# wuji3/visiondk

Hardware: AMD Instinct MI355X
Metric: images/sec fwd+bwd+optimizer step (ViT-B/16, bs=256 per GPU) (higher is better)
Workload: dtype fp16; 1 GPU; ViT-B/16 ICT, synthetic ImageNet-1k 224x224, random-init weights (reference re-init), per-GPU batch 256, CE label_smoothing 0.05, SGD 0.006/0.937/5e-4, clip 10, EMA on rank 0; global_batch=256, parallelism=dp1

## Files before the change

visiondk_amd/csrc/vit_engine.hip:

```cpp
#include <hip/hip_runtime.h>
#include <stdlib.h>
#include <stdio.h>
#include <string.h>
#include "vdk_device.h"
#include "vdk_host.h"
#include "vdk_gemm.h"

extern "C" {
int vdk_layernorm_fwd(const float*, int64_t, int32_t, int32_t, const float*, const float*, float, void*, int64_t, int32_t, float*, float*, void*);
int vdk_layernorm_bwd_workspace_bytes(int32_t, int32_t, size_t*);
int vdk_layernorm_bwd(const void*, int64_t, int32_t, const float*, int64_t, const float*, const float*, const float*, const float*, int64_t,
                      int32_t, int32_t, float*, int64_t, void*, int64_t, float*, float*, void*, size_t, void*);
int vdk_reduce_rows_f32(const float*, int64_t, int32_t, int64_t, float*, float, void*);
int vdk_colsum_bf16_workspace_bytes(int32_t, int32_t, size_t*);
int vdk_colsum_bf16(const void*, int64_t, int32_t, int32_t, float*, void*, size_t, void*);
int vdk_attention_fwd(const void*, int64_t, void*, int64_t, float*, int32_t, int32_t, int32_t, int32_t, float, void*);
int vdk_attention_bwd(const void*, int64_t, const void*, const void*, int64_t, const float*, void*, int64_t, float*, int32_t, int32_t, int32_t,
                      int32_t, float, void*);
int vdk_attention_fwd_dt(const void*, int64_t, void*, int64_t, float*, int32_t, int32_t, int32_t, int32_t, float, int32_t, void*);
int vdk_attention_bwd_dt(const void*, int64_t, const void*, const void*, int64_t, const float*, void*, int64_t, float*, int32_t, int32_t, int32_t, int32_t, float, int32_t, void*);
int vdk_attention_bwd_cs(const void*, int64_t, const void*, const void*, int64_t, const float*, void*, int64_t, float*, int32_t, int32_t, int32_t, int32_t, float, int32_t, float*, int32_t*,
                         void*);
int vdk_patchify_bf16(const float*, int32_t, int32_t, int32_t, int32_t, int32_t, void*, int32_t, void*);
int vdk_cls_rows(float*, int64_t, int32_t, int32_t, const float*, const float*, void*);
int vdk_cast_f32_bf16(const float*, void*, int64_t, void*);
int vdk_transpose_cast_f32_bf16(const float*, int64_t, int32_t, int32_t, void*, int64_t, int32_t, void*);
int vdk_gemm_f32_nt(const VdkGemmF32Desc*, void*);
int vdk_gemm_a_colsum_rows(int32_t, int32_t, int32_t);
int vdk_softmax_rows_f32(float*, int64_t, int64_t, int32_t, float, void*);
int vdk_patchify_f32(const float*, int32_t, int32_t, int32_t, int32_t, int32_t, float*, void*);
int vdk_quant_fp8(const void*, int32_t, int64_t, const float*, void*, int32_t, float*, void*);
int vdk_fp8_scale_update(float*, float*, float*, int32_t, int32_t, float, void*);
int vdk_gemm_fp8_nt(const VdkGemmDesc*, int32_t, int32_t, const float*, const float*, void*);
int vdk_gemm_fp8_nt_q8(const VdkGemmDesc*, int32_t, int32_t, const float*, const float*, void*, int64_t, int32_t, const float*, float*, void*);
int vdk_layernorm_fwd_q8(const float*, int64_t, int32_t, int32_t, const float*, const float*, float, void*, int64_t, float*, float*, void*, int64_t, int32_t, const float*, float*, void*);
}


static thread_local int t_opf = VDK_OPF_BF16;
#define DT16 (t_opf ? VDK_F16 : VDK_BF16)
static bool gelu_saved_grad() {
  static const int v = [] { const char* e = getenv("VDK_VIT_GELU_SAVED_GRAD"); return e ? atoi(e) : -1; }();
  return v < 0 ? t_opf != 0 : v != 0;
}
#define ACT_FC1 (gelu_saved_grad() ? VDK_ACT_GELU_SAVE_GRAD : VDK_ACT_GELU)
#define ACT_DFC2 (gelu_saved_grad() ? VDK_ACT_MUL_AUX : VDK_ACT_DGELU)

static inline int64_t up(int64_t x, int64_t a) { return (x + a - 1) / a * a; }

struct VitDims {
  int B, img, ps, Cin, D, L, H, M, C, Cp, np, N, T, Kraw, Kpe, Tp, Bp, cls, pre , fp8, opf ;
  float eps;
};
static int vit_dims(const VdkVitConfig* c, VitDims* d) {
  if (!c) return vdk_fail(VDK_EINVAL, "vit: null config");
  d->B = c->batch; d->img = c->img_size; d->ps = c->patch_size; d->Cin = c->in_chans; d->D = c->dim; d->L = c->depth;
  d->H = c->heads; d->M = c->mlp_dim; d->C = c->num_classes; d->eps = c->ln_eps;
  if (d->B <= 0 || d->img <= 0 || d->ps <= 0 || d->img % d->ps || d->Cin <= 0 || d->D <= 0 || d->L <= 0 || d->H <= 0 || d->M <= 0 || d->C < 0)
    return vdk_fail(VDK_EINVAL, "vit: bad config value");
  if (d->D != d->H * 64) return vdk_fail(VDK_EUNSUPPORTED, "vit: head_dim must be 64 (dim == 64 * heads)");
  if ((d->D & 7) || (d->M & 7)) return vdk_fail(VDK_EUNSUPPORTED, "vit: dim and mlp_dim must be multiples of 8");
  d->Kraw = d->Cin * d->ps * d->ps;
  d->Kpe = (int)up(d->Kraw, 8);
  d->np = (d->img / d->ps) * (d->img / d->ps);
  d->cls = c->no_class_token ? 0 : 1;
  d->pre = c->pre_norm ? 1 : 0;
  if (d->pre && c->fp8) return vdk_fail(VDK_EUNSUPPORTED, "vit: pre_norm and the fp8 mode are not combined");
  if (!d->cls && d->C > 0) return vdk_fail(VDK_EUNSUPPORTED, "vit: no_class_token is feature mode only (num_classes == 0)");
  d->N = d->np + d->cls;
// ... 144 lines not shown
  if (s > 64) s = 64;
  if (s < 1) s = 1;
  return s;
}
static int vit_plan(const VitDims& d, WsPlan* w) {
  size_t cur = 0;
  const size_t T = d.T, D = d.D, M = d.M, L = d.L;
  w->patches = w_take(cur, (size_t)d.B * d.np * d.Kpe * 2);
  w->pepad = w->dwpe = 0;
  if (d.Kraw != d.Kpe) { w->pepad = w_take(cur, D * d.Kpe * 2); w->dwpe = w_take(cur, D * d.Kpe * 4); }
  w->X = w_take(cur, (2 * L + 1) * T * D * 4);
  w->xe = w->pstats = 0;
  if (d.pre) { w->xe = w_take(cur, T * D * 4); w->pstats = w_take(cur, 2 * T * 4); }
  w->stats = w_take(cur, (L * 4 * T + 2 * T) * 4);
  w->s_h = T * D * 2; w->s_qkv = T * 3 * D * 2; w->s_lse = (size_t)d.B * d.H * d.N * 4; w->s_u = T * M * 2;
  w->h1 = w_take(cur, L * w->s_h); w->qkv = w_take(cur, L * w->s_qkv); w->lse = w_take(cur, L * w->s_lse);
  w->o = w_take(cur, L * w->s_h); w->h2 = w_take(cur, L * w->s_h); w->u = w_take(cur, L * w->s_u); w->g = w_take(cur, L * w->s_u);
  w->hf = w_take(cur, (size_t)d.Bp * D * 2);
  w->dxa = w_take(cur, T * D * 4); w->dxm = w_take(cur, T * D * 4);
  size_t big = M > 3 * D ? M : 3 * D;
  for (int i = 0; i < 3; ++i) w->dxab[i] = w_take(cur, T * D * 2);
  for (int i = 0; i < 2; ++i) {
    w->dxmb[i] = w_take(cur, T * D * 2);
    w->du[i] = w_take(cur, T * M * 2); w->dqkv[i] = w_take(cur, T * 3 * D * 2);
  }
  w->dsm = w_take(cur, T * D * 2);
  w->dvec = w_take(cur, w->s_lse);
  size_t trows = big > (size_t)d.Cp ? big : (size_t)d.Cp;
  if (trows < (size_t)d.Kpe) trows = d.Kpe;
  size_t tcols = d.Tp > d.Bp ? d.Tp : d.Bp;
  w->tA = w_take(cur, trows * tcols * 2); w->tB = w_take(cur, trows * tcols * 2);
  size_t sl = 0;
  {
    int sh[5][3] = {{(int)M, (int)D, d.T}, {(int)D, (int)M, d.T}, {3 * (int)D, (int)D, d.T}, {(int)D, (int)D, d.T}, {(int)D, d.Kpe, d.B * d.np}};
    for (auto& s : sh) {
      int k1 = wgrad_splitk(s[0], s[1], s[2]), k2 = wgrad_splitk_tn(s[0], s[1], s[2]);
      size_t b = (size_t)(k1 > k2 ? k1 : k2) * s[0] * s[1] * 4; if (b > sl) sl = b;
    }
  }
  w->slabs_bytes = sl; w->slabs = w_take(cur, sl);
  vdk_layernorm_bwd_workspace_bytes(d.T, d.D, &w->lnws_bytes); w->lnws_bytes = (w->lnws_bytes + 255) & ~(size_t)255; w->lnws = w_take(cur, 2 * w->lnws_bytes);
  size_t cs = (size_t)((tcols + 63) / 64) * trows * 4;
  { size_t cs2 = 0; vdk_colsum_bf16_workspace_bytes(d.T, (int)trows, &cs2); if (cs2 > cs) cs = cs2; }
  { size_t cs3 = (size_t)2 * ((d.T + 255) / 256) * trows * 4; if (cs3 > cs) cs = cs3; }
  w->csws_bytes = (cs + 255) & ~(size_t)255; w->csws = w_take(cur, 5 * w->csws_bytes);
  w->dhf = w_take(cur, (size_t)d.B * D * 2);
  w->dposall = w_take(cur, (size_t)d.N * D * 4);
  w->a8 = d.fp8 ? w_take(cur, T * (M > 3 * D ? M : 3 * D)) : 0;
  w->a8b = d.fp8 ? w_take(cur, T * M) : 0;
  w->total = cur;
  return VDK_OK;
}

#define RC(x) do { int rc_ = (x); if (rc_) return rc_; } while (0)

static bool cls_tail_on(const VitDims& d) {
  const char* e = getenv("VDK_VIT_CLS_TAIL");
  return d.C > 0 && d.cls && !d.fp8 && !(e && e[0] == '0');
}

struct F8 {
  int mode; unsigned char* w8; unsigned char* wt8; float* amax; float* sc; float* si; unsigned char* a8; unsigned char* a8b;
};
static int f8_init(const VdkVitConfig* cfg, const VitDims& d, const PLayout& p, F8* f, unsigned char* a8, unsigned char* a8b) {
  f->mode = d.fp8; f->a8 = a8; f->a8b = a8b;
  if (!d.fp8) return VDK_OK;
  if (!cfg->fp8_w || !cfg->fp8_state) return vdk_fail(VDK_EINVAL, "vit: fp8 mode without fp8_w / fp8_state");
  if (a8 && d.T < 256) return vdk_fail(VDK_EUNSUPPORTED, "vit: the fp8 mode needs batch * tokens >= 256");
  f->w8 = (unsigned char*)cfg->fp8_w; f->wt8 = f->w8 + p.total;
  const int S = 12 * d.L;
  f->amax = cfg->fp8_state; f->sc = f->amax + S; f->si = f->sc + S;
  return VDK_OK;
}
static int f8_quant(hipStream_t s, const F8& f, const void* x, int xdt, long n, int slot, int fmt, unsigned char* out, int force_current = 0) {
  if (f.mode == 2 || force_current) {
    RC(vdk_quant_fp8(x, xdt, n, nullptr, nullptr, fmt, f.amax + slot, s));
    RC(vdk_fp8_scale_update(f.amax + slot, f.sc + slot, f.si + slot, 1, fmt, 1.0f, s));
  }
  return vdk_quant_fp8(x, xdt, n, f.sc + slot, out, fmt, f.amax + slot, s);
}
static bool f8_fused(const F8& f) {
  const char* e = getenv("VDK_FP8_FUSED_QUANT");
  return f.mode == 1 && !(e && e[0] == '0');
}
static int gemm8(hipStream_t s, const F8& f, const void* a, int slot_a, int a_fmt, const unsigned char* w8, int slot_w, int64_t ldb, void* Cc, int64_t ldc, int M, int N,
                 int K, int cdt, const float* bias, const float* res, int64_t ldr, int act, void* aux, int64_t ldaux, const unsigned char* a_pre = nullptr, int q8_slot = -1,
                 int q8_fmt = 0, float* c_colsum = nullptr) {
  if (!a_pre) RC(f8_quant(s, f, a, VDK_BF16, (long)M * K, slot_a, a_fmt, f.a8));
  VdkGemmDesc g = {};
  g.A = a_pre ? a_pre : f.a8; g.lda = K; g.B = w8; g.ldb = ldb; g.C = Cc; g.ldc = ldc; g.M = M; g.N = N; g.K = K; g.c_dtype = cdt; g.bias = bias; g.residual = res; g.ldr = ldr;
  g.act = act; g.aux = aux; g.ldaux = ldaux; g.alpha = 1.0f; g.splitk = 1; g.c_colsum = c_colsum;
// ... 117 lines not shown
                    float* logits, void* stream_) {
  hipStream_t s = (hipStream_t)stream_;
  VitDims d; RC(vit_dims(cfg, &d));
  PLayout p; RC(vit_layout(d, &p));
  WsPlan w; RC(vit_plan(d, &w));
  if (!x || !params || !wb16 || !ws || !logits) return vdk_fail(VDK_EINVAL, "vdk_vit_forward: null pointer");
  if (ws_bytes < w.total) return vdk_fail(VDK_EWORKSPACE, "vdk_vit_forward: workspace too small");
  t_opf = d.opf;
  char* base = (char*)ws;
  const bf16_t* wb = (const bf16_t*)wb16;
  const int T = d.T, D = d.D, M = d.M;
  float* X = (float*)(base + w.X);
  float* stats = (float*)(base + w.stats);
  const size_t XS = (size_t)T * D;

  bf16_t* patches = (bf16_t*)(base + w.patches);
  RC(vdk_patchify_16(x, d.B, d.Cin, d.img, d.img, d.ps, patches, d.Kpe, t_opf, s));
  const bf16_t* pew = wb + p.pe_w;
  if (d.Kraw != d.Kpe) {
    RC(vdk_cast_pad_rows(params + p.pe_w, d.Kraw, D, d.Kraw, base + w.pepad, d.Kpe, s, t_opf));
    pew = (const bf16_t*)(base + w.pepad);
  }
  float* const X0 = d.pre ? (float*)(base + w.xe) : X;
  RC(gemm(s, patches, d.Kpe, pew, d.Kpe, X0, D, d.B * d.np, D, d.Kpe, VDK_F32, params + p.pe_b, params + p.pos, D, VDK_ACT_NONE,
          nullptr, 0, 1, d.cls ? d.np : -d.np, nullptr, 0));
  if (d.cls) RC(vdk_cls_rows(X0, (int64_t)d.N * D, d.B, D, params + p.cls, params + p.pos, s));
  if (d.pre) {
    float* ps = (float*)(base + w.pstats);
    RC(vdk_layernorm_fwd(X0, D, T, D, params + p.npre_w, params + p.npre_b, d.eps, X, D, VDK_F32, ps, ps + T, s));
  }

  const float scale = 0.125f;
  F8 f8; RC(f8_init(cfg, d, p, &f8, (unsigned char*)(base + w.a8), (unsigned char*)(base + w.a8b)));
  const bool cls_tail = cls_tail_on(d);
  for (int l = 0; l < d.L; ++l) {
    const PLayout::Blk& b = p.blk[l];
    float* xin = X + (size_t)(2 * l) * XS; float* xmid = xin + XS; float* xout = xmid + XS;
    float* mean1 = stats + (size_t)l * 4 * T; float* rstd1 = mean1 + T; float* mean2 = rstd1 + T; float* rstd2 = mean2 + T;
    bf16_t* h1 = (bf16_t*)(base + w.h1 + l * w.s_h); bf16_t* qkv = (bf16_t*)(base + w.qkv + l * w.s_qkv);
    float* lse = (float*)(base + w.lse + l * w.s_lse); bf16_t* o = (bf16_t*)(base + w.o + l * w.s_h);
    bf16_t* h2 = (bf16_t*)(base + w.h2 + l * w.s_h); bf16_t* u = (bf16_t*)(base + w.u + l * w.s_u); bf16_t* g = (bf16_t*)(base + w.g + l * w.s_u);
    if (f8.mode) {
      const int sl = 12 * l;
      const bool fl = f8_fused(f8) && D > 128 && D <= 1024, fq = f8_fused(f8) && (M % 64) == 0;
      if (fl) RC(vdk_layernorm_fwd_q8(xin, D, T, D, params + b.n1w, params + b.n1b, d.eps, h1, D, mean1, rstd1, f8.a8, D, 0, f8.sc + sl + 0, f8.amax + sl + 0, s));
      else RC(vdk_layernorm_fwd(xin, D, T, D, params + b.n1w, params + b.n1b, d.eps, h1, D, VDK_BF16, mean1, rstd1, s));
      RC(gemm8(s, f8, h1, sl + 0, 0, f8.w8 + b.qkv_w, sl + 4, D, qkv, 3 * D, T, 3 * D, D, VDK_BF16, params + b.qkv_b, nullptr, 0, VDK_ACT_NONE, nullptr, 0, fl ? f8.a8 : nullptr));
      RC(vdk_attention_fwd(qkv, 3 * D, o, D, lse, d.B, d.N, d.H, 64, scale, s));
      RC(gemm8(s, f8, o, sl + 1, 0, f8.w8 + b.proj_w, sl + 5, D, xmid, D, T, D, D, VDK_F32, params + b.proj_b, xin, D, VDK_ACT_NONE, nullptr, 0));
      if (fl) RC(vdk_layernorm_fwd_q8(xmid, D, T, D, params + b.n2w, params + b.n2b, d.eps, h2, D, mean2, rstd2, f8.a8, D, 0, f8.sc + sl + 2, f8.amax + sl + 2, s));
      else RC(vdk_layernorm_fwd(xmid, D, T, D, params + b.n2w, params + b.n2b, d.eps, h2, D, VDK_BF16, mean2, rstd2, s));
      RC(gemm8(s, f8, h2, sl + 2, 0, f8.w8 + b.fc1_w, sl + 6, D, g, M, T, M, D, VDK_BF16, params + b.fc1_b, nullptr, 0, VDK_ACT_GELU, u, M, fl ? f8.a8 : nullptr, fq ? sl + 3 : -1, 0));
      RC(gemm8(s, f8, g, sl + 3, 0, f8.w8 + b.fc2_w, sl + 7, M, xout, D, T, D, M, VDK_F32, params + b.fc2_b, xmid, D, VDK_ACT_NONE, nullptr, 0, fq ? f8.a8b : nullptr));
      continue;
    }
    RC(vdk_layernorm_fwd(xin, D, T, D, params + b.n1w, params + b.n1b, d.eps, h1, D, DT16, mean1, rstd1, s));
    RC(gemm(s, h1, D, wb + b.qkv_w, D, qkv, 3 * D, T, 3 * D, D, DT16, params + b.qkv_b, nullptr, 0, VDK_ACT_NONE, nullptr, 0, 1, 0, nullptr, 0));
    RC(vdk_attention_fwd_dt(qkv, 3 * D, o, D, lse, d.B, d.N, d.H, 64, scale, DT16, s));
    const bool tail = cls_tail && l == d.L - 1;
    const int R = tail ? d.B : T;
    const int64_t ldt = tail ? (int64_t)d.N * D : D;
    RC(gemm(s, o, ldt, wb + b.proj_w, D, xmid, ldt, R, D, D, VDK_F32, params + b.proj_b, xin, ldt, VDK_ACT_NONE, nullptr, 0, 1, 0, nullptr, 0));
    RC(vdk_layernorm_fwd(xmid, ldt, R, D, params + b.n2w, params + b.n2b, d.eps, h2, D, DT16, mean2, rstd2, s));
    RC(gemm(s, h2, D, wb + b.fc1_w, D, g, M, R, M, D, DT16, params + b.fc1_b, nullptr, 0, ACT_FC1, u, M, 1, 0, nullptr, 0));
    RC(gemm(s, g, M, wb + b.fc2_w, M, xout, ldt, R, D, M, VDK_F32, params + b.fc2_b, xmid, ldt, VDK_ACT_NONE, nullptr, 0, 1, 0, nullptr, 0));
  }
  float* xl = X + (size_t)(2 * d.L) * XS;
  float* meanf = stats + (size_t)d.L * 4 * T; float* rstdf = meanf + T;
  if (d.C == 0) {
    RC(vdk_layernorm_fwd(xl, D, T, D, params + p.norm_w, params + p.norm_b, d.eps, logits, D, VDK_F32, meanf, rstdf, s));
    return VDK_OK;
  }
  bf16_t* hf = (bf16_t*)(base + w.hf);
  RC(vdk_layernorm_fwd(xl, (int64_t)d.N * D, d.B, D, params + p.norm_w, params + p.norm_b, d.eps, hf, D, DT16, meanf, rstdf, s));
  RC(gemm(s, hf, D, wb + p.head_w, D, logits, d.Cp, d.B, d.Cp, D, VDK_F32, params + p.head_b, nullptr, 0, VDK_ACT_NONE, nullptr, 0, 1, 0, nullptr, 0));
  return VDK_OK;
}

static int linear_wgrad(hipStream_t s, const VitDims& d, const WsPlan& w, char* base, const bf16_t* dY, int64_t lddy, const bf16_t* Xa,
                        int64_t ldx, int rows, int rows_pad, int out, int in, float* dW, float* db, int dy_row_group) {
  if ((rows % 64) == 0 && (out % 8) == 0 && (in % 8) == 0 && out >= 8 && in >= 8 && !(t_opf && dy_row_group != 0)) {
    const int sk = wgrad_splitk_tn(out, in, rows);
    VdkGemmDesc g = {};
    g.A = dY; g.lda = lddy; g.B = Xa; g.ldb = ldx; g.C = dW; g.ldc = in; g.M = out; g.N = in; g.K = rows; g.c_dtype = VDK_F32;
    g.alpha = 1.0f; g.splitk = sk; g.trans = 1; g.a_row_group = dy_row_group; g.ab_dtype = DT16;
    RC(vdk_gemm_bf16_nt(&g, base + w.slabs, w.slabs_bytes, s));
    if (db && dy_row_group == 0) RC(vdk_colsum_16(dY, lddy, rows, out, db, base + w.csws + 4 * w.csws_bytes, w.csws_bytes, t_opf, s));
    return VDK_OK;
  }
  bf16_t* tA = (bf16_t*)(base + w.tA); bf16_t* tB = (bf16_t*)(base + w.tB);
  float* csp = (db && dy_row_group == 0) ? (float*)(base + w.csws + 4 * w.csws_bytes) : nullptr;
// ... 32 lines not shown
  RC(vdk_gemm_bf16_nt(&g, nullptr, 0, s));
  if (*fused) jobs[(*njobs)++] = VdkReduceJob{part, (long)out, prow, (long)out, db, 1.0f};
  if (fx) jobs[(*njobs)++] = VdkReduceJob{partx, (long)in, xrow, (long)in, dbx, 1.0f};
  return VDK_OK;
}

int vdk_vit_backward(const VdkVitConfig* cfg, const void* dlogits, const float* params, const void* wb16, const void* wt16, void* ws,
                     size_t ws_bytes, float* grads, vdk_grad_ready_fn on_ready, void* user, void* stream_, void* side_stream_) {
  hipStream_t s = (hipStream_t)stream_;
  hipStream_t s2 = side_stream_ ? (hipStream_t)side_stream_ : s;
  VitDims d; RC(vit_dims(cfg, &d));
  PLayout p; RC(vit_layout(d, &p));
  WsPlan w; RC(vit_plan(d, &w));
  if (!dlogits || !params || !wb16 || !wt16 || !ws || !grads) return vdk_fail(VDK_EINVAL, "vdk_vit_backward: null pointer");
  if (ws_bytes < w.total) return vdk_fail(VDK_EWORKSPACE, "vdk_vit_backward: workspace too small");
  t_opf = d.opf;
  char* base = (char*)ws;
  const bf16_t* wt = (const bf16_t*)wt16;
  const int T = d.T, D = d.D, M = d.M;
  float* X = (float*)(base + w.X);
  float* stats = (float*)(base + w.stats);
  const size_t XS = (size_t)T * D;
  float* dxa = (float*)(base + w.dxa); float* dxm = (float*)(base + w.dxm);
#define DXAB(l) ((bf16_t*)(base + w.dxab[((l) + 3) % 3]))
#define DXMB(l) ((bf16_t*)(base + w.dxmb[((l) + 2) & 1]))
#define DU(l) ((bf16_t*)(base + w.du[((l) + 2) & 1]))
#define DQKV(l) ((bf16_t*)(base + w.dqkv[((l) + 2) & 1]))
  bf16_t* dsm = (bf16_t*)(base + w.dsm);
  float* dvec = (float*)(base + w.dvec);
  void* lnws = base + w.lnws;
  const size_t EV_SIDE_DONE = 8;
  size_t ev_p = EV_SIDE_DONE + d.L + 4;
  RC(ev_order(0, s, s2));
  const bool cls_tail = cls_tail_on(d);

  bool last_fc2_bias_done = false;
  if (d.C == 0) {
    float* xl = X + (size_t)(2 * d.L) * XS;
    float* meanf = stats + (size_t)d.L * 4 * T; float* rstdf = meanf + T;
    RC(vdk_layernorm_bwd_deferred(dlogits, D, VDK_F32, xl, D, meanf, rstdf, params + p.norm_w, nullptr, 0, T, D, dxa, D, DXAB(d.L - 1), D, grads + p.norm_w,
                                  grads + p.norm_b, lnws, w.lnws_bytes, s, nullptr, nullptr, nullptr, nullptr, t_opf));
    if (on_ready) on_ready(user, p.norm_w, p.total - p.norm_w);
  } else {
    const bf16_t* dl = (const bf16_t*)dlogits;
    bf16_t* hf = (bf16_t*)(base + w.hf);
    RC(linear_wgrad(s, d, w, base, dl, d.Cp, hf, D, d.B, d.Bp, d.Cp, D, grads + p.head_w, grads + p.head_b, 0));
    bf16_t* dhf = (bf16_t*)(base + w.dhf);
    RC(gemm(s, dl, d.Cp, wt + p.headT, d.Cp, dhf, D, d.B, D, d.Cp, DT16, nullptr, nullptr, 0, VDK_ACT_NONE, nullptr, 0, 1, 0, nullptr, 0));
    if (!cls_tail && (hipMemsetAsync(dxa, 0, XS * 4, s) != hipSuccess || hipMemsetAsync(DXAB(d.L - 1), 0, XS * 2, s) != hipSuccess))
      return vdk_fail(VDK_ELAUNCH, "vdk_vit_backward: memset failed");
    float* xl = X + (size_t)(2 * d.L) * XS;
    float* meanf = stats + (size_t)d.L * 4 * T; float* rstdf = meanf + T;
    if (s2 == s && D <= 1024) {
      VdkReduceJob fj[2];
      RC(vdk_layernorm_bwd_deferred(dhf, D, DT16, xl, (int64_t)d.N * D, meanf, rstdf, params + p.norm_w, nullptr, 0, d.B, D, dxa, (int64_t)d.N * D, DXAB(d.L - 1),
                                    (int64_t)d.N * D, grads + p.norm_w, grads + p.norm_b, lnws, w.lnws_bytes, s, &fj[0], grads + p.blk[d.L - 1].fc2_b, &fj[1]));
      if (fj[0].in) RC(vdk_reduce_rows_batch(fj, 2, s)); else RC(vdk_reduce_rows_batch(fj + 1, 1, s));
      last_fc2_bias_done = true;
    } else
    RC(vdk_layernorm_bwd(dhf, D, DT16, xl, (int64_t)d.N * D, meanf, rstdf, params + p.norm_w, nullptr, 0, d.B, D, dxa, (int64_t)d.N * D, DXAB(d.L - 1),
                         (int64_t)d.N * D, grads + p.norm_w, grads + p.norm_b, lnws, w.lnws_bytes, s));
    if (on_ready) on_ready(user, p.norm_w, p.total - p.norm_w);
  }
  bool fc2_bias_from_norm1 = false, dxab8_ready = false;
  F8 f8; RC(f8_init(cfg, d, p, &f8, (unsigned char*)(base + w.a8), (unsigned char*)(base + w.a8b)));
  for (int l = d.L - 1; l >= 0; --l) {
    const PLayout::Blk& b = p.blk[l];
    float* xin = X + (size_t)(2 * l) * XS; float* xmid = xin + XS;
    float* mean1 = stats + (size_t)l * 4 * T; float* rstd1 = mean1 + T; float* mean2 = rstd1 + T; float* rstd2 = mean2 + T;
    bf16_t* h1 = (bf16_t*)(base + w.h1 + l * w.s_h); bf16_t* qkv = (bf16_t*)(base + w.qkv + l * w.s_qkv);
    float* lse = (float*)(base + w.lse + l * w.s_lse); bf16_t* o = (bf16_t*)(base + w.o + l * w.s_h);
    bf16_t* h2 = (bf16_t*)(base + w.h2 + l * w.s_h); bf16_t* u = (bf16_t*)(base + w.u + l * w.s_u); bf16_t* g = (bf16_t*)(base + w.g + l * w.s_u);
    bf16_t* dxab = DXAB(l); bf16_t* dxmb = DXMB(l); bf16_t* du = DU(l); bf16_t* dqkv = DQKV(l);
    if (s2 != s && l + 2 <= d.L - 1) { hipEvent_t e; RC(ev_get(EV_SIDE_DONE + l + 3, &e)); if (hipStreamWaitEvent(s, e, 0) != hipSuccess) return vdk_fail(VDK_ELAUNCH, "vit: wait failed"); }
    int fz = 0;
    const bool one_stream = (s2 == s);
    VdkReduceJob jobs[8]; int nj = 0;
    char* const lnws0 = base + w.lnws; char* const lnws1 = lnws0 + w.lnws_bytes;
    const bool ocs_ln = one_stream && D <= 1024;
    static const bool g16_on = !(getenv("VDK_VIT_G16") && atoi(getenv("VDK_VIT_G16")) == 0);
    const bool g16 = g16_on && ocs_ln && !f8.mode && t_opf == VDK_OPF_F16 && D > 512 && D <= 1024;
    const bool tail = cls_tail && l == d.L - 1;
    const int R = tail ? d.B : T, Rp = tail ? d.Bp : d.Tp;
    const int64_t ldt = tail ? (int64_t)d.N * D : D;
    if (tail && (hipMemsetAsync(dsm, 0, XS * 2, s) != hipSuccess || (g16 ? hipMemsetAsync(dxmb, 0, XS * 2, s) : hipMemsetAsync(dxm, 0, XS * 4, s)) != hipSuccess))
      return vdk_fail(VDK_ELAUNCH, "vdk_vit_backward: memset failed");
    RC(ev_order(ev_p++, s, s2));
    if (f8.mode) {
      const int sl = 12 * l;
      const bool have_fc2b = one_stream && ((l == d.L - 1) ? last_fc2_bias_done : fc2_bias_from_norm1);
      const bool fq = f8_fused(f8) && (M % 64) == 0;
      const int xrow = one_stream ? 2 * ((T + 255) / 256) : 0;
      const bool fo = xrow > 0 && (size_t)xrow * M * 4 <= w.csws_bytes;
      float* const partx = (float*)(base + w.csws + (size_t)1 * w.csws_bytes);
      RC(gemm8(s, f8, dxab, sl + 8, 1, f8.wt8 + p.blkT[l].fc2, sl + 7, D, du, M, T, M, D, VDK_BF16, nullptr, nullptr, 0, VDK_ACT_DGELU, u, M, dxab8_ready ? f8.a8 : nullptr,
               fq ? sl + 9 : -1, 1, fo ? partx : nullptr));
      if (fo) jobs[nj++] = VdkReduceJob{partx, (long)M, xrow, (long)M, grads + b.fc1_b, 1.0f};
      RC(linear_wgrad(s2, d, w, base, dxab, D, g, M, T, d.Tp, D, M, grads + b.fc2_w, have_fc2b ? nullptr : grads + b.fc2_b, 0));
      RC(gemm8(s, f8, du, sl + 9, 1, f8.wt8 + p.blkT[l].fc1, sl + 6, M, dsm, D, T, D, M, VDK_BF16, nullptr, nullptr, 0, VDK_ACT_NONE, nullptr, 0, fq ? f8.a8b : nullptr));
      RC(linear_wgrad(s2, d, w, base, du, M, h2, D, T, d.Tp, M, D, grads + b.fc1_w, fo ? nullptr : grads + b.fc1_b, 0));
    } else if (one_stream) {
      int fx = 0;
      const bool have_fc2b = (l == d.L - 1) ? last_fc2_bias_done : fc2_bias_from_norm1;
      RC(dgrad_with_bias(s, w, base, dxab, ldt, wt + p.blkT[l].fc2, D, du, M, R, M, D, ACT_DFC2, u, M, have_fc2b ? nullptr : grads + b.fc2_b, &fz, 0, jobs, &nj,
                         grads + b.fc1_b, &fx, 1));
      RC(linear_wgrad(s2, d, w, base, dxab, ldt, g, M, R, Rp, D, M, grads + b.fc2_w, (fz || have_fc2b) ? nullptr : grads + b.fc2_b, 0));
      if (fx) {
        RC(gemm(s, du, M, wt + p.blkT[l].fc1, M, dsm, ldt, R, D, M, DT16, nullptr, nullptr, 0, VDK_ACT_NONE, nullptr, 0, 1, 0, nullptr, 0));
        fz = 1;
      } else {
        RC(dgrad_with_bias(s, w, base, du, M, wt + p.blkT[l].fc1, M, dsm, ldt, R, D, M, VDK_ACT_NONE, nullptr, 0, grads + b.fc1_b, &fz, 1, jobs, &nj));
      }
      RC(linear_wgrad(s2, d, w, base, du, M, h2, D, R, Rp, M, D, grads + b.fc1_w, fz ? nullptr : grads + b.fc1_b, 0));
    } else {
      RC(linear_wgrad(s2, d, w, base, dxab, ldt, g, M, R, Rp, D, M, grads + b.fc2_w, grads + b.fc2_b, 0));
      RC(gemm(s, dxab, ldt, wt + p.blkT[l].fc2, D, du, M, R, M, D, DT16, nullptr, nullptr, 0, ACT_DFC2, u, M, 1, 0, nullptr, 0));
      RC(ev_order(ev_p++, s, s2));
      RC(linear_wgrad(s2, d, w, base, du, M, h2, D, R, Rp, M, D, grads + b.fc1_w, grads + b.fc1_b, 0));
      RC(gemm(s, du, M, wt + p.blkT[l].fc1, M, dsm, ldt, R, D, M, DT16, nullptr, nullptr, 0, VDK_ACT_NONE, nullptr, 0, 1, 0, nullptr, 0));
    }
    const bool lq = f8.mode && f8_fused(f8) && ocs_ln;
    const LnQ8 q8m = {f8.a8, (long)D, f8.sc + 12 * l + 10, f8.amax + 12 * l + 10, 1};
    if (g16) RC(vdk_layernorm_bwd_deferred(dsm, ldt, DT16, xmid, ldt, mean2, rstd2, params + b.n2w, nullptr, ldt, R, D, nullptr, ldt, dxmb, ldt, grads + b.n2w, grads + b.n2b, lnws0,
                                           w.lnws_bytes, s, &jobs[nj], grads + b.proj_b, &jobs[nj + 1], nullptr, 0, nullptr, nullptr, 1, dxab));
    else
    RC(vdk_layernorm_bwd_deferred(dsm, ldt, DT16, xmid, ldt, mean2, rstd2, params + b.n2w, dxa, ldt, R, D, dxm, ldt, dxmb, ldt, grads + b.n2w, grads + b.n2b, lnws0,
                                  w.lnws_bytes, s, &jobs[nj], ocs_ln ? grads + b.proj_b : nullptr, ocs_ln ? &jobs[nj + 1] : nullptr, lq ? &q8m : nullptr));
    nj += ocs_ln ? 2 : 1;
    RC(ev_order(ev_p++, s, s2));
    if (f8.mode) {
      RC(gemm8(s, f8, dxmb, 12 * l + 10, 1, f8.wt8 + p.blkT[l].proj, 12 * l + 5, D, dsm, D, T, D, D, VDK_BF16, nullptr, nullptr, 0, VDK_ACT_NONE, nullptr, 0, lq ? f8.a8 : nullptr));
      RC(linear_wgrad(s2, d, w, base, dxmb, D, o, D, T, d.Tp, D, D, grads + b.proj_w, ocs_ln ? nullptr : grads + b.proj_b, 0));
    } else if (one_stream && ocs_ln) {
      RC(gemm(s, dxmb, ldt, wt + p.blkT[l].proj, D, dsm, ldt, R, D, D, DT16, nullptr, nullptr, 0, VDK_ACT_NONE, nullptr, 0, 1, 0, nullptr, 0));
      RC(linear_wgrad(s2, d, w, base, dxmb, ldt, o, ldt, R, Rp, D, D, grads + b.proj_w, nullptr, 0));
    } else if (one_stream) {
      RC(dgrad_with_bias(s, w, base, dxmb, ldt, wt + p.blkT[l].proj, D, dsm, ldt, R, D, D, VDK_ACT_NONE, nullptr, 0, grads + b.proj_b, &fz, 2, jobs, &nj));
      RC(linear_wgrad(s2, d, w, base, dxmb, ldt, o, ldt, R, Rp, D, D, grads + b.proj_w, fz ? nullptr : grads + b.proj_b, 0));
    } else {
      RC(linear_wgrad(s2, d, w, base, dxmb, ldt, o, ldt, R, Rp, D, D, grads + b.proj_w, grads + b.proj_b, 0));
      RC(gemm(s, dxmb, ldt, wt + p.blkT[l].proj, D, dsm, ldt, R, D, D, DT16, nullptr, nullptr, 0, VDK_ACT_NONE, nullptr, 0, 1, 0, nullptr, 0));
    }
    int32_t qkvb_done = 0;
    {
      static const bool fuse_on = !(getenv("VDK_VIT_QKVB_ATTN") && atoi(getenv("VDK_VIT_QKVB_ATTN")) == 0);
      float* csp = (fuse_on && !f8.mode && one_stream && (size_t)d.B * 3 * D * 4 <= w.csws_bytes) ? (float*)(base + w.csws + (size_t)3 * w.csws_bytes) : nullptr;
      RC(vdk_attention_bwd_cs(qkv, 3 * D, o, dsm, D, lse, dqkv, 3 * D, dvec, d.B, d.N, d.H, 64, 0.125f, DT16, csp, &qkvb_done, s));
      if (qkvb_done) { jobs[nj] = VdkReduceJob{csp, (long)3 * D, d.B, (long)3 * D, grads + b.qkv_b, 1.0f}; ++nj; }
    }
    RC(ev_order(ev_p++, s, s2));
    if (f8.mode) {
      size_t csneed = 0; vdk_colsum_bf16_workspace_bytes(T, 3 * D, &csneed);
      const bool fcq = f8_fused(f8) && one_stream && csneed <= w.csws_bytes;
      if (fcq) {
        const LnQ8 q8d = {f8.a8, (long)3 * D, f8.sc + 12 * l + 11, f8.amax + 12 * l + 11, 1};
        RC(vdk_colsum_bf16_deferred(dqkv, 3 * D, T, 3 * D, grads + b.qkv_b, base + w.csws + (size_t)2 * w.csws_bytes, w.csws_bytes, s, &jobs[nj], &q8d)); ++nj;
      }
      RC(gemm8(s, f8, dqkv, 12 * l + 11, 1, f8.wt8 + p.blkT[l].qkv, 12 * l + 4, 3 * D, dsm, D, T, D, 3 * D, VDK_BF16, nullptr, nullptr, 0, VDK_ACT_NONE, nullptr, 0,
               fcq ? f8.a8 : nullptr));
      RC(linear_wgrad(s2, d, w, base, dqkv, 3 * D, h1, D, T, d.Tp, 3 * D, D, grads + b.qkv_w, fcq ? nullptr : grads + b.qkv_b, 0));
    } else if (one_stream && (qkvb_done || qkvb_pass(T, 3 * D, w.csws_bytes))) {
      if (!qkvb_done) { RC(vdk_colsum_bf16_deferred(dqkv, 3 * D, T, 3 * D, grads + b.qkv_b, base + w.csws + (size_t)3 * w.csws_bytes, w.csws_bytes, s, &jobs[nj], nullptr, t_opf)); ++nj; }
      RC(gemm(s, dqkv, 3 * D, wt + p.blkT[l].qkv, 3 * D, dsm, D, T, D, 3 * D, DT16, nullptr, nullptr, 0, VDK_ACT_NONE, nullptr, 0, 1, 0, nullptr, 0));
      RC(linear_wgrad(s2, d, w, base, dqkv, 3 * D, h1, D, T, d.Tp, 3 * D, D, grads + b.qkv_w, nullptr, 0));
    } else if (one_stream) {
      RC(dgrad_with_bias(s, w, base, dqkv, 3 * D, wt + p.blkT[l].qkv, 3 * D, dsm, D, T, D, 3 * D, VDK_ACT_NONE, nullptr, 0, grads + b.qkv_b, &fz, 3, jobs, &nj));
      RC(linear_wgrad(s2, d, w, base, dqkv, 3 * D, h1, D, T, d.Tp, 3 * D, D, grads + b.qkv_w, fz ? nullptr : grads + b.qkv_b, 0));
    } else {
      RC(linear_wgrad(s2, d, w, base, dqkv, 3 * D, h1, D, T, d.Tp, 3 * D, D, grads + b.qkv_w, grads + b.qkv_b, 0));
      RC(gemm(s, dqkv, 3 * D, wt + p.blkT[l].qkv, 3 * D, dsm, D, T, D, 3 * D, DT16, nullptr, nullptr, 0, VDK_ACT_NONE, nullptr, 0, 1, 0, nullptr, 0));
    }
    const bool ocs_n1 = ocs_ln && l > 0;
    const bool lq1 = lq && ocs_n1;
    const LnQ8 q8a = {f8.a8, (long)D, f8.sc + 12 * (l - 1) + 8, f8.amax + 12 * (l - 1) + 8, 1};
    if (g16 && l > 0) RC(vdk_layernorm_bwd_deferred(dsm, D, DT16, xin, D, mean1, rstd1, params + b.n1w, nullptr, D, T, D, nullptr, D, DXAB(l - 1), D, grads + b.n1w, grads + b.n1b, lnws1,
                                                    w.lnws_bytes, s, &jobs[nj], grads + p.blk[l - 1].fc2_b, &jobs[nj + 1], nullptr, 0, nullptr, nullptr, 1, dxmb));
    else if (g16) {
      float* const dummy_cs = (float*)(base + w.csws);
      RC(vdk_layernorm_bwd_deferred(dsm, D, DT16, xin, D, mean1, rstd1, params + b.n1w, nullptr, D, T, D, dxa, D, DXAB(l - 1), D, grads + b.n1w, grads + b.n1b, lnws1,
                                    w.lnws_bytes, s, &jobs[nj], dummy_cs, &jobs[nj + 1], nullptr, 0, nullptr, nullptr, 1, dxmb));
    } else
    RC(vdk_layernorm_bwd_deferred(dsm, D, DT16, xin, D, mean1, rstd1, params + b.n1w, dxm, D, T, D, dxa, D, DXAB(l - 1), D, grads + b.n1w, grads + b.n1b, lnws1,
                                  w.lnws_bytes, s, &jobs[nj], ocs_n1 ? grads + p.blk[l - 1].fc2_b : nullptr, ocs_n1 ? &jobs[nj + 1] : nullptr, lq1 ? &q8a : nullptr));
    dxab8_ready = lq1;
// ... 134 lines not shown
```

Before: 7748 images/sec.

## Compute only CLS query in last ViT block attention forward and backward

In the last transformer block, where only the CLS token output feeds the classifier tail, the QKV projection computes Q only for CLS rows (K,V for all tokens). A new dedicated single-query attention kernel handles forward and backward, and the backward dgrad/wgrad GEMMs are split into a full K/V part and a CLS-only Q part. This removes redundant Q projection, full NxN attention, and Q-gradient GEMM work for non-CLS tokens, at the cost of extra small GEMM launches and a new hand-written kernel.

```diff
diff --git a/visiondk_amd/csrc/attention_cls.hip b/visiondk_amd/csrc/attention_cls.hip
--- /dev/null
+++ b/visiondk_amd/csrc/attention_cls.hip
@@ -0,0 +1,214 @@
+#include <hip/hip_runtime.h>
+#include <stdlib.h>
+#include <math.h>
+#include "vdk_device.h"
+#include "vdk_host.h"
+
+#define AC_U 4
+#define AC_WAVES 4
+
+template <int OF> __device__ __forceinline__ void ac_unpack(const u32x4& v, float (&f)[8]) {
+#pragma unroll
+  for (int e = 0; e < 4; ++e) { f[2 * e] = op_lo<OF>(v[e]); f[2 * e + 1] = op_hi<OF>(v[e]); }
+}
+__device__ __forceinline__ float ac_dot(const float (&a)[8], const float (&b)[8]) {
+  float d = 0.f;
+#pragma unroll
+  for (int e = 0; e < 8; ++e) d = fmaf(a[e], b[e], d);
+  return d;
+}
+__device__ __forceinline__ float ac_row_sum(float d) { d += __shfl_xor(d, 1); d += __shfl_xor(d, 2); d += __shfl_xor(d, 4); return d; }
+__device__ __forceinline__ float ac_col_sum(float d) { d += __shfl_xor(d, 8); d += __shfl_xor(d, 16); d += __shfl_xor(d, 32); return d; }
+
+template <int OF>
+__global__ __launch_bounds__(64 * AC_WAVES) void attn_cls_fwd_kernel(const bf16_t* __restrict__ qkv, long ld, bf16_t* __restrict__ o, long ldo, float* __restrict__ lse, int N, int H,
+                                                                      float scale, int nitems, int nwaves) {
+  VDK_DYN_LDS(smem);
+  const int tid = threadIdx.x, lane = tid & 63, r = lane >> 3, c = lane & 7;
+  const int w = __builtin_amdgcn_readfirstlane(tid >> 6);
+  const int NS = (N + 63) & ~63;
+  float* const S = (float*)smem + (size_t)w * NS;
+  const long D = (long)H * 64;
+  const float scale2 = scale * VDK_LOG2E;
+  for (int item = blockIdx.x * nwaves + w; item < nitems; item += gridDim.x * nwaves) {
+    const int b = item / H, h = item - b * H;
+    const bf16_t* const qp = qkv + (long)b * N * ld + h * 64;
+    const bf16_t* const kp = qp + D + c * 8;
+    const bf16_t* const vp = qp + 2 * D + c * 8;
+    float qf[8];
+    ac_unpack<OF>(*(const u32x4*)(qp + c * 8), qf);
+    float m = -INFINITY;
+    for (int j0 = 0; j0 < N; j0 += 8 * AC_U) {
+      u32x4 kv[AC_U];
+#pragma unroll
+      for (int u = 0; u < AC_U; ++u) {
+        const int row = j0 + 8 * u + r;
+        kv[u] = (u32x4){0u, 0u, 0u, 0u};
+        if (row < N) kv[u] = *(const u32x4*)(kp + (long)row * ld);
+      }
+#pragma unroll
+      for (int u = 0; u < AC_U; ++u) {
+        const int row = j0 + 8 * u + r;
+        float kf[8];
+        ac_unpack<OF>(kv[u], kf);
+        const float s = ac_row_sum(ac_dot(qf, kf));
+        if (row < N) { m = fmaxf(m, s); if (c == 0) S[row] = s; }
+      }
+    }
+    m = fmaxf(m, __shfl_xor(m, 8)); m = fmaxf(m, __shfl_xor(m, 16)); m = fmaxf(m, __shfl_xor(m, 32));
+    const float m2 = m * scale2;
+    VDK_WAVE_LDS_SYNC();
+    float l = 0.f;
+    for (int j = lane; j < NS; j += 64)
+      if (j < N) { const float p = fast_exp2(fmaf(S[j], scale2, -m2)); S[j] = p; l += p; }
+    l = ac_col_sum(ac_row_sum(l));
+    const float inv = 1.0f / l;
+    VDK_WAVE_LDS_SYNC();
+    float acc[8] = {0.f, 0.f, 0.f, 0.f, 0.f, 0.f, 0.f, 0.f};
+    for (int j0 = 0; j0 < N; j0 += 8 * AC_U) {
+      u32x4 vv[AC_U];
+#pragma unroll
+      for (int u = 0; u < AC_U; ++u) {
+        const int row = j0 + 8 * u + r;
+        vv[u] = (u32x4){0u, 0u, 0u, 0u};
+        if (row < N) vv[u] = *(const u32x4*)(vp + (long)row * ld);
+      }
+#pragma unroll
+      for (int u = 0; u < AC_U; ++u) {
+        const int row = j0 + 8 * u + r;
+        float vf[8];
+        ac_unpack<OF>(vv[u], vf);
+        const float p16 = row < N ? op2f<OF>(f2op<OF>(S[row] * inv)) : 0.f;
+#pragma unroll
+        for (int e = 0; e < 8; ++e) acc[e] = fmaf(p16, vf[e], acc[e]);
+      }
+    }
+#pragma unroll
+    for (int e = 0; e < 8; ++e) acc[e] = ac_col_sum(acc[e]);
+    if (r == 0)
+      *(u32x4*)(o + (long)b * N * ldo + h * 64 + c * 8) = (u32x4){pack_op2<OF>(acc[0], acc[1]), pack_op2<OF>(acc[2], acc[3]), pack_op2<OF>(acc[4], acc[5]), pack_op2<OF>(acc[6], acc[7])};
+    if (lane == 0) lse[((long)b * H + h) * N] = (m2 + log2f(l)) * 0.6931471805599453f;
+    VDK_WAVE_LDS_SYNC();
+  }
+}
+
+template <int OF>
+__global__ __launch_bounds__(64 * AC_WAVES) void attn_cls_bwd_kernel(const bf16_t* __restrict__ qkv, long ld, const bf16_t* __restrict__ o, const bf16_t* __restrict__ dout, long ldo,
+                                                                      const float* __restrict__ lse, bf16_t* __restrict__ dqkv, long ldd, float* __restrict__ cspart, int N, int H,
+                                                                      float scale, int nitems) {
+  const int tid = threadIdx.x, lane = tid & 63, r = lane >> 3, c = lane & 7;
+  const int w = __builtin_amdgcn_readfirstlane(tid >> 6);
+  const long D = (long)H * 64;
+  const float scale2 = scale * VDK_LOG2E;
+  for (int item = blockIdx.x * AC_WAVES + w; item < nitems; item += gridDim.x * AC_WAVES) {
+    const int b = item / H, h = item - b * H;
+    const bf16_t* const qp = qkv + (long)b * N * ld + h * 64;
+    const bf16_t* const kp = qp + D + c * 8;
+    const bf16_t* const vp = qp + 2 * D + c * 8;
+    bf16_t* const dqp = dqkv + (long)b * N * ldd + h * 64 + c * 8;
+    bf16_t* const dkp = dqp + D;
+    bf16_t* const dvp = dqp + 2 * D;
+    float qf[8], gf[8];
+    ac_unpack<OF>(*(const u32x4*)(qp + c * 8), qf);
+    const u32x4 g4 = *(const u32x4*)(dout + (long)b * N * ldo + h * 64 + c * 8);
+    const u32x4 o4 = *(const u32x4*)(o + (long)b * N * ldo + h * 64 + c * 8);
+    ac_unpack<OF>(g4, gf);
+    float Dd = 0.f;
+#pragma unroll
+    for (int e = 0; e < 4; ++e) { Dd = fmaf(op_lo<OF>(g4[e]), op_lo<OF>(o4[e]), Dd); Dd = fmaf(op_hi<OF>(g4[e]), op_hi<OF>(o4[e]), Dd); }
+    Dd = ac_row_sum(Dd);
+    const float lse2 = lse[((long)b * H + h) * N] * VDK_LOG2E;
+    float dqa[8], csk[8], csv[8];
+#pragma unroll
+    for (int e = 0; e < 8; ++e) { dqa[e] = 0.f; csk[e] = 0.f; csv[e] = 0.f; }
+    for (int j0 = 0; j0 < N; j0 += 8 * AC_U) {
+      u32x4 kv[AC_U], vv[AC_U];
+#pragma unroll
+      for (int u = 0; u < AC_U; ++u) {
+        const int row = j0 + 8 * u + r;
+        kv[u] = (u32x4){0u, 0u, 0u, 0u}; vv[u] = (u32x4){0u, 0u, 0u, 0u};
+        if (row < N) { kv[u] = *(const u32x4*)(kp + (long)row * ld); vv[u] = *(const u32x4*)(vp + (long)row * ld); }
+      }
+#pragma unroll
+      for (int u = 0; u < AC_U; ++u) {
+        const int row = j0 + 8 * u + r;
+        float kf[8], vf[8];
+        ac_unpack<OF>(kv[u], kf);
+        ac_unpack<OF>(vv[u], vf);
+        const float s = ac_row_sum(ac_dot(qf, kf));
+        const float dp = ac_row_sum(ac_dot(gf, vf));
+        if (row < N) {
+          const float p = fast_exp2(fmaf(s, scale2, -lse2));
+          const float p16 = op2f<OF>(f2op<OF>(p)), ds16 = op2f<OF>(f2op<OF>(p * (dp - Dd)));
+          u32x4 dk4, dv4;
+#pragma unroll
+          for (int e = 0; e < 4; ++e) {
+            dk4[e] = pack_op2<OF>(ds16 * qf[2 * e] * scale, ds16 * qf[2 * e + 1] * scale);
+            dv4[e] = pack_op2<OF>(p16 * gf[2 * e], p16 * gf[2 * e + 1]);
+            csk[2 * e] += op_lo<OF>(dk4[e]); csk[2 * e + 1] += op_hi<OF>(dk4[e]);
+            csv[2 * e] += op_lo<OF>(dv4[e]); csv[2 * e + 1] += op_hi<OF>(dv4[e]);
+          }
+          *(u32x4*)(dkp + (long)row * ldd) = dk4;
+          *(u32x4*)(dvp + (long)row * ldd) = dv4;
+#pragma unroll
+          for (int e = 0; e < 8; ++e) dqa[e] = fmaf(ds16, kf[e], dqa[e]);
+        }
+      }
+    }
+#pragma unroll
+    for (int e = 0; e < 8; ++e) { dqa[e] = ac_col_sum(dqa[e]); csk[e] = ac_col_sum(csk[e]); csv[e] = ac_col_sum(csv[e]); }
+    if (r == 0) {
+      const u32x4 dq4 = {pack_op2<OF>(dqa[0] * scale, dqa[1] * scale), pack_op2<OF>(dqa[2] * scale, dqa[3] * scale), pack_op2<OF>(dqa[4] * scale, dqa[5] * scale),
+                         pack_op2<OF>(dqa[6] * scale, dqa[7] * scale)};
+      *(u32x4*)dqp = dq4;
+      float* const cq = cspart + (((long)b * 3 + 0) * H + h) * 64 + c * 8;
+      float* const ck = cspart + (((long)b * 3 + 1) * H + h) * 64 + c * 8;
+      float* const cv = cspart + (((long)b * 3 + 2) * H + h) * 64 + c * 8;
+      *(f32x4*)cq = (f32x4){op_lo<OF>(dq4[0]), op_hi<OF>(dq4[0]), op_lo<OF>(dq4[1]), op_hi<OF>(dq4[1])};
+      *(f32x4*)(cq + 4) = (f32x4){op_lo<OF>(dq4[2]), op_hi<OF>(dq4[2]), op_lo<OF>(dq4[3]), op_hi<OF>(dq4[3])};
+      *(f32x4*)ck = (f32x4){csk[0], csk[1], csk[2], csk[3]}; *(f32x4*)(ck + 4) = (f32x4){csk[4], csk[5], csk[6], csk[7]};
+      *(f32x4*)cv = (f32x4){csv[0], csv[1], csv[2], csv[3]}; *(f32x4*)(cv + 4) = (f32x4){csv[4], csv[5], csv[6], csv[7]};
+    }
+  }
+}
+
+static int ac_grid(int nitems, int nwaves) {
+  int grid = (nitems + nwaves - 1) / nwaves;
+  if (const char* e = getenv("VDK_ATTN_CLS_GRID")) { const int v = atoi(e); if (v > 0 && v < grid) grid = v; }
+  return grid;
+}
+static int ac_check(const void* qkv, int64_t ld, int64_t ldo, int32_t B, int32_t N, int32_t H) {
+  if (!qkv || B <= 0 || N <= 0 || H <= 0) return vdk_fail(VDK_EINVAL, "attn_cls: bad argument");
+  if ((ld & 7) || (ldo & 7) || ((uintptr_t)qkv & 15)) return vdk_fail(VDK_EINVAL, "attn_cls: rows must be 16-byte aligned");
+  return VDK_OK;
+}
+
+int vdk_attn_cls_fwd(const void* qkv, int64_t ld, void* o, int64_t ldo, float* lse, int32_t B, int32_t N, int32_t H, float scale, int opf, void* stream) {
+  if (int rc = ac_check(qkv, ld, ldo, B, N, H)) return rc;
+  if (!o || !lse || ((uintptr_t)o & 15)) return vdk_fail(VDK_EINVAL, "attn_cls_fwd: bad argument");
+  const size_t per_wave = (size_t)((N + 63) & ~63) * 4;
+  const int nwaves = per_wave * AC_WAVES <= 32768 ? AC_WAVES : 1;
+  if (per_wave * nwaves > 160 * 1024) return vdk_fail(VDK_EUNSUPPORTED, "attn_cls_fwd: more than 40960 tokens");
+  const size_t lds = per_wave * nwaves;
+  hipStream_t s = (hipStream_t)stream;
+  const int nitems = B * H, grid = ac_grid(nitems, nwaves);
+  const void* fn = opf ? (const void*)attn_cls_fwd_kernel<VDK_OPF_F16> : (const void*)attn_cls_fwd_kernel<VDK_OPF_BF16>;
+  if (lds > 65536 && hipFuncSetAttribute(fn, hipFuncAttributeMaxDynamicSharedMemorySize, (int)lds) != hipSuccess) return vdk_fail(VDK_ELAUNCH, "attn_cls_fwd: LDS attribute");
+  if (opf) hipLaunchKernelGGL((attn_cls_fwd_kernel<VDK_OPF_F16>), dim3((unsigned)grid), dim3(64 * nwaves), lds, s, (const bf16_t*)qkv, (long)ld, (bf16_t*)o, (long)ldo, lse, N, H, scale, nitems, nwaves);
+  else hipLaunchKernelGGL((attn_cls_fwd_kernel<VDK_OPF_BF16>), dim3((unsigned)grid), dim3(64 * nwaves), lds, s, (const bf16_t*)qkv, (long)ld, (bf16_t*)o, (long)ldo, lse, N, H, scale, nitems, nwaves);
+  return vdk_check_launch("attn_cls_fwd");
+}
+
+int vdk_attn_cls_bwd(const void* qkv, int64_t ld, const void* o, const void* dout, int64_t ldo, const float* lse, void* dqkv, int64_t ldd, float* cspart, int32_t B, int32_t N,
+                     int32_t H, float scale, int opf, void* stream) {
+  if (int rc = ac_check(qkv, ld, ldo, B, N, H)) return rc;
+  if (!o || !dout || !lse || !dqkv || !cspart || (ldd & 7) || (((uintptr_t)o | (uintptr_t)dout | (uintptr_t)dqkv | (uintptr_t)cspart) & 15))
+    return vdk_fail(VDK_EINVAL, "attn_cls_bwd: bad argument");
+  hipStream_t s = (hipStream_t)stream;
+  const int nitems = B * H, grid = ac_grid(nitems, AC_WAVES);
+  if (opf) hipLaunchKernelGGL((attn_cls_bwd_kernel<VDK_OPF_F16>), dim3((unsigned)grid), dim3(64 * AC_WAVES), 0, s, (const bf16_t*)qkv, (long)ld, (const bf16_t*)o, (const bf16_t*)dout, (long)ldo, lse,
+                              (bf16_t*)dqkv, (long)ldd, cspart, N, H, scale, nitems);
+  else hipLaunchKernelGGL((attn_cls_bwd_kernel<VDK_OPF_BF16>), dim3((unsigned)grid), dim3(64 * AC_WAVES), 0, s, (const bf16_t*)qkv, (long)ld, (const bf16_t*)o, (const bf16_t*)dout, (long)ldo, lse,
+                          (bf16_t*)dqkv, (long)ldd, cspart, N, H, scale, nitems);
+  return vdk_check_launch("attn_cls_bwd");
+}
diff --git a/visiondk_amd/csrc/vit_engine.hip b/visiondk_amd/csrc/vit_engine.hip
--- a/visiondk_amd/csrc/vit_engine.hip
+++ b/visiondk_amd/csrc/vit_engine.hip
@@ -35,6 +35,9 @@
 int vdk_gemm_fp8_nt_q8(const VdkGemmDesc*, int32_t, int32_t, const float*, const float*, void*, int64_t, int32_t, const float*, float*, void*);
 int vdk_layernorm_fwd_q8(const float*, int64_t, int32_t, int32_t, const float*, const float*, float, void*, int64_t, float*, float*, void*, int64_t, int32_t, const float*, float*, void*);
 }
+int vdk_attn_cls_fwd(const void* qkv, int64_t ld, void* o, int64_t ldo, float* lse, int32_t B, int32_t N, int32_t H, float scale, int opf, void* stream);
+int vdk_attn_cls_bwd(const void* qkv, int64_t ld, const void* o, const void* dout, int64_t ldo, const float* lse, void* dqkv, int64_t ldd, float* cspart, int32_t B, int32_t N,
+                     int32_t H, float scale, int opf, void* stream);
 
 
 static thread_local int t_opf = VDK_OPF_BF16;
@@ -245,7 +248,8 @@
   w->tA = w_take(cur, trows * tcols * 2); w->tB = w_take(cur, trows * tcols * 2);
   size_t sl = 0;
   {
-    int sh[5][3] = {{(int)M, (int)D, d.T}, {(int)D, (int)M, d.T}, {3 * (int)D, (int)D, d.T}, {(int)D, (int)D, d.T}, {(int)D, d.Kpe, d.B * d.np}};
+    int sh[6][3] = {{(int)M, (int)D, d.T}, {(int)D, (int)M, d.T}, {3 * (int)D, (int)D, d.T}, {(int)D, (int)D, d.T}, {(int)D, d.Kpe, d.B * d.np},
+                    {2 * (int)D, (int)D, d.T} };
     for (auto& s : sh) {
       int k1 = wgrad_splitk(s[0], s[1], s[2]), k2 = wgrad_splitk_tn(s[0], s[1], s[2]);
       size_t b = (size_t)(k1 > k2 ? k1 : k2) * s[0] * s[1] * 4; if (b > sl) sl = b;
@@ -270,6 +274,10 @@
 static bool cls_tail_on(const VitDims& d) {
   const char* e = getenv("VDK_VIT_CLS_TAIL");
   return d.C > 0 && d.cls && !d.fp8 && !(e && e[0] == '0');
+}
+static bool cls_query_on(const VitDims& d, const WsPlan& w) {
+  const char* e = getenv("VDK_VIT_CLS_QUERY");
+  return cls_tail_on(d) && !(e && e[0] == '0') && (size_t)d.B * 3 * d.D * 4 <= w.csws_bytes;
 }
 
 struct F8 {
@@ -453,7 +461,7 @@
 
   const float scale = 0.125f;
   F8 f8; RC(f8_init(cfg, d, p, &f8, (unsigned char*)(base + w.a8), (unsigned char*)(base + w.a8b)));
-  const bool cls_tail = cls_tail_on(d);
+  const bool cls_tail = cls_tail_on(d), cls_query = cls_query_on(d, w);
   for (int l = 0; l < d.L; ++l) {
     const PLayout::Blk& b = p.blk[l];
     float* xin = X + (size_t)(2 * l) * XS; float* xmid = xin + XS; float* xout = xmid + XS;
@@ -476,8 +484,14 @@
       continue;
     }
     RC(vdk_layernorm_fwd(xin, D, T, D, params + b.n1w, params + b.n1b, d.eps, h1, D, DT16, mean1, rstd1, s));
-    RC(gemm(s, h1, D, wb + b.qkv_w, D, qkv, 3 * D, T, 3 * D, D, DT16, params + b.qkv_b, nullptr, 0, VDK_ACT_NONE, nullptr, 0, 1, 0, nullptr, 0));
-    RC(vdk_attention_fwd_dt(qkv, 3 * D, o, D, lse, d.B, d.N, d.H, 64, scale, DT16, s));
+    if (cls_query && l == d.L - 1) {
+      RC(gemm(s, h1, D, wb + b.qkv_w + (size_t)D * D, D, qkv + D, 3 * D, T, 2 * D, D, DT16, params + b.qkv_b + D, nullptr, 0, VDK_ACT_NONE, nullptr, 0, 1, 0, nullptr, 0));
+      RC(gemm(s, h1, (int64_t)d.N * D, wb + b.qkv_w, D, qkv, (int64_t)d.N * 3 * D, d.B, D, D, DT16, params + b.qkv_b, nullptr, 0, VDK_ACT_NONE, nullptr, 0, 1, 0, nullptr, 0));
+      RC(vdk_attn_cls_fwd(qkv, 3 * D, o, D, lse, d.B, d.N, d.H, scale, t_opf, s));
+    } else {
+      RC(gemm(s, h1, D, wb + b.qkv_w, D, qkv, 3 * D, T, 3 * D, D, DT16, params + b.qkv_b, nullptr, 0, VDK_ACT_NONE, nullptr, 0, 1, 0, nullptr, 0));
+      RC(vdk_attention_fwd_dt(qkv, 3 * D, o, D, lse, d.B, d.N, d.H, 64, scale, DT16, s));
+    }
     const bool tail = cls_tail && l == d.L - 1;
     const int R = tail ? d.B : T;
     const int64_t ldt = tail ? (int64_t)d.N * D : D;
@@ -576,7 +590,7 @@
   const size_t EV_SIDE_DONE = 8;
   size_t ev_p = EV_SIDE_DONE + d.L + 4;
   RC(ev_order(0, s, s2));
-  const bool cls_tail = cls_tail_on(d);
+  const bool cls_tail = cls_tail_on(d), cls_query = cls_query_on(d, w);
 
   bool last_fc2_bias_done = false;
   if (d.C == 0) {
@@ -624,10 +638,10 @@
     const bool ocs_ln = one_stream && D <= 1024;
     static const bool g16_on = !(getenv("VDK_VIT_G16") && atoi(getenv("VDK_VIT_G16")) == 0);
     const bool g16 = g16_on && ocs_ln && !f8.mode && t_opf == VDK_OPF_F16 && D > 512 && D <= 1024;
-    const bool tail = cls_tail && l == d.L - 1;
+    const bool tail = cls_tail && l == d.L - 1, cq = tail && cls_query;
     const int R = tail ? d.B : T, Rp = tail ? d.Bp : d.Tp;
     const int64_t ldt = tail ? (int64_t)d.N * D : D;
-    if (tail && (hipMemsetAsync(dsm, 0, XS * 2, s) != hipSuccess || (g16 ? hipMemsetAsync(dxmb, 0, XS * 2, s) : hipMemsetAsync(dxm, 0, XS * 4, s)) != hipSuccess))
+    if (tail && ((!cq && hipMemsetAsync(dsm, 0, XS * 2, s) != hipSuccess) || (g16 ? hipMemsetAsync(dxmb, 0, XS * 2, s) : hipMemsetAsync(dxm, 0, XS * 4, s)) != hipSuccess))
       return vdk_fail(VDK_ELAUNCH, "vdk_vit_backward: memset failed");
     RC(ev_order(ev_p++, s, s2));
     if (f8.mode) {
@@ -686,14 +700,23 @@
       RC(gemm(s, dxmb, ldt, wt + p.blkT[l].proj, D, dsm, ldt, R, D, D, DT16, nullptr, nullptr, 0, VDK_ACT_NONE, nullptr, 0, 1, 0, nullptr, 0));
     }
     int32_t qkvb_done = 0;
-    {
+    if (cq) {
+      float* csp = (float*)(base + w.csws + (size_t)3 * w.csws_bytes);
+      RC(vdk_attn_cls_bwd(qkv, 3 * D, o, dsm, D, lse, dqkv, 3 * D, csp, d.B, d.N, d.H, 0.125f, t_opf, s));
+      jobs[nj++] = VdkReduceJob{csp, (long)3 * D, d.B, (long)3 * D, grads + b.qkv_b, 1.0f};
+    } else {
       static const bool fuse_on = !(getenv("VDK_VIT_QKVB_ATTN") && atoi(getenv("VDK_VIT_QKVB_ATTN")) == 0);
       float* csp = (fuse_on && !f8.mode && one_stream && (size_t)d.B * 3 * D * 4 <= w.csws_bytes) ? (float*)(base + w.csws + (size_t)3 * w.csws_bytes) : nullptr;
       RC(vdk_attention_bwd_cs(qkv, 3 * D, o, dsm, D, lse, dqkv, 3 * D, dvec, d.B, d.N, d.H, 64, 0.125f, DT16, csp, &qkvb_done, s));
       if (qkvb_done) { jobs[nj] = VdkReduceJob{csp, (long)3 * D, d.B, (long)3 * D, grads + b.qkv_b, 1.0f}; ++nj; }
     }
     RC(ev_order(ev_p++, s, s2));
-    if (f8.mode) {
+    if (cq) {
+      RC(gemm(s, dqkv + D, 3 * D, wt + p.blkT[l].qkv + D, 3 * D, dsm, D, T, D, 2 * D, DT16, nullptr, nullptr, 0, VDK_ACT_NONE, nullptr, 0, 1, 0, nullptr, 0));
+      RC(gemm(s, dqkv, (int64_t)d.N * 3 * D, wt + p.blkT[l].qkv, 3 * D, dsm, (int64_t)d.N * D, d.B, D, 3 * D, DT16, nullptr, nullptr, 0, VDK_ACT_NONE, nullptr, 0, 1, 0, nullptr, 0));
+      RC(linear_wgrad(s2, d, w, base, dqkv + D, 3 * D, h1, D, T, d.Tp, 2 * D, D, grads + b.qkv_w + (size_t)D * D, nullptr, 0));
+      RC(linear_wgrad(s2, d, w, base, dqkv, (int64_t)d.N * 3 * D, h1, (int64_t)d.N * D, d.B, d.Bp, D, D, grads + b.qkv_w, nullptr, 0));
+    } else if (f8.mode) {
       size_t csneed = 0; vdk_colsum_bf16_workspace_bytes(T, 3 * D, &csneed);
       const bool fcq = f8_fused(f8) && one_stream && csneed <= w.csws_bytes;
       if (fcq) {
```

Result: no change. 7809 images/sec (median of 6 runs) (+0.8%).
